# Julian-Wyatt/AnoDDPM

Hardware: AMD Instinct MI355X
Metric: reverse-diffusion images/sec @256x256 T=1000 simplex (higher is better)
Workload: dtype f32; 1 GPU; 256x256 simplex(8 oct) T=1000 base128 attn16,8 batch4/GPU (BASELINE config 2); per_gpu_batch=4, global_batch=4, T=1000, parallelism=batch-sharded x1 (no data-path collective), output_finite=True

## Files before the change

### anoddpm_amd/csrc/executor.hip

```cpp
#include <stdarg.h>
#include <string.h>
#include <vector>
#include "common.h"

namespace anoddpm {

static thread_local char g_err[512] = "";
int g_debug[16] = {0};

void set_error(const char *fmt, ...)
{
    va_list ap;
    va_start(ap, fmt);
    vsnprintf(g_err, sizeof(g_err), fmt, ap);
    va_end(ap);
}

struct ProfState {
    bool on = false;
    std::vector<hipEvent_t> pool;
    std::vector<int> codes;
    std::vector<float> last_ms;
    std::vector<int> last_codes;
    size_t used = 0;
// ... 7 lines not shown
    X(GN_STATS,         anoddpm_gn_args,               anoddpm_gn_stats) \
    X(SOFTMAX,          anoddpm_softmax_args,          anoddpm_softmax_rows) \
    X(RESAMPLE,         anoddpm_resample_args,         anoddpm_resample2x) \
    X(LINEAR,           anoddpm_linear_args,           anoddpm_linear_small) \
    X(POSEMB,           anoddpm_posemb_args,           anoddpm_posemb) \
    X(STEM,             anoddpm_stem_args,             anoddpm_conv_stem) \
    X(LAYOUT,           anoddpm_layout_args,           anoddpm_nhwc_to_nchw) \
    X(CHAN_STATS,       anoddpm_chan_stats_args,       anoddpm_chan_stats) \
    X(HEAD,             anoddpm_head_args,             anoddpm_conv_head) \
    X(GN_FINALIZE,      anoddpm_gn_finalize_args,      anoddpm_gn_finalize) \
    X(WGRAD3,           anoddpm_wgrad_args,            anoddpm_conv3x3_wgrad) \
    X(WGRAD1,           anoddpm_wgrad1_args,           anoddpm_wgrad_pointwise) \
    X(GN_BWD,           anoddpm_gn_bwd_args,           anoddpm_gn_silu_backward) \
    X(PACK,             anoddpm_pack_args,             anoddpm_pack_weights) \
    X(SOFTMAX_BWD,      anoddpm_softmax_bwd_args,      anoddpm_softmax_rows_backward) \
    X(TRANSPOSE,        anoddpm_transpose_args,        anoddpm_transpose_square) \
    X(LINEAR_BWD,       anoddpm_linear_bwd_args,       anoddpm_linear_small_backward) \
    X(STEM_BWD,         anoddpm_stem_bwd_args,         anoddpm_conv_stem_backward) \
    X(HEAD_BWD,         anoddpm_head_bwd_args,         anoddpm_conv_head_backward) \
    X(COLSUM_FOLD,      anoddpm_colsum_fold_args,      anoddpm_colsum_fold) \
    X(ATTENTION,        anoddpm_attention_args,        anoddpm_attention) \
    X(PACK_BATCH,       anoddpm_pack_batch_args,       anoddpm_pack_batch) \
    X(DROPOUT,          anoddpm_dropout_args,          anoddpm_dropout) \
    X(LINEAR_BWD_BATCH, anoddpm_linear_bwd_batch_args, anoddpm_linear_small_backward_batch)

static int dispatch(const anoddpm_op &op, void *stream)
{
    switch (op.code) {
#define X(code, args_t, fn) case ANODDPM_OP_##code: return fn(static_cast<const args_t *>(op.args), stream);
        ANODDPM_OPS(X)
#undef X
        default: set_error("run_ops: unknown op code %d", op.code); return ANODDPM_EINVAL;
    }
}

}

using namespace anoddpm;

extern "C" int anoddpm_internal_variant(int32_t key, int32_t value)
{
    if (key < 0 || key >= 16) return ANODDPM_EINVAL;
#ifndef ANODDPM_ABLATE
    if (!(key == 0 || key == 4 || key == 5 || key == 8 || key == 9)) {
        set_error("internal_variant: key %d selects a timing ablation; this library was built without ANODDPM_ABLATE", key);
        return ANODDPM_EINVAL;
    }
// ... 98 lines not shown
extern "C" int anoddpm_prof_list(int32_t *codes, float *ms, int32_t cap)
{
    const int n = (int)g_prof.last_ms.size();
    for (int i = 0; i < n && i < cap; ++i) {
        if (codes) codes[i] = g_prof.last_codes[i];
        if (ms) ms[i] = g_prof.last_ms[i];
    }
    return n;
}

#define ANODDPM_STRUCTS(X) \
    X(anoddpm_simplex_args) X(anoddpm_p_update_args) X(anoddpm_igemm_args) X(anoddpm_gn_args) X(anoddpm_softmax_args) \
    X(anoddpm_resample_args) X(anoddpm_linear_args) X(anoddpm_posemb_args) X(anoddpm_stem_args) X(anoddpm_layout_args) \
    X(anoddpm_op) X(anoddpm_adamw_args) X(anoddpm_chan_stats_args) X(anoddpm_gn_finalize_args) X(anoddpm_head_args) \
    X(anoddpm_anomaly_args) X(anoddpm_vlb_args) X(anoddpm_wgrad_args) X(anoddpm_gn_bwd_args) X(anoddpm_wgrad1_args) \
    X(anoddpm_pack_args) X(anoddpm_softmax_bwd_args) X(anoddpm_transpose_args) X(anoddpm_linear_bwd_args) \
    X(anoddpm_stem_bwd_args) X(anoddpm_head_bwd_args) X(anoddpm_colsum_fold_args) X(anoddpm_mri_slice_args) \
    X(anoddpm_resize_args) X(anoddpm_attention_args) X(anoddpm_pack_batch_args) X(anoddpm_linear_bwd_batch_args) \
    X(anoddpm_loss_args) X(anoddpm_dropout_args) X(anoddpm_roc_args) X(anoddpm_ssim_args) X(anoddpm_component_areas_args) \
    X(anoddpm_pro_args) X(anoddpm_distance_args) X(anoddpm_surface_args) X(anoddpm_median_args) X(anoddpm_erode_args) \
    X(anoddpm_components_args) X(anoddpm_gauss_args) X(anoddpm_map_scores_args) \
    X(anoddpm_ano_slices_args) X(anoddpm_select_args) X(anoddpm_threshold_counts_args) X(anoddpm_known_args) \
    X(anoddpm_resampling_args) X(anoddpm_keep_mask_args) X(anoddpm_median3d_args) X(anoddpm_erode3d_args) \
    X(anoddpm_components3d_args) X(anoddpm_component_areas3d_args) X(anoddpm_distance3d_args) X(anoddpm_surface3d_args)

extern "C" int anoddpm_struct_size(const char *name)
{
    if (reinterpret_cast<uintptr_t>(name) < 4096) return -1;
#define X(s) if (strcmp(name, #s) == 0) return (int)sizeof(s);
    ANODDPM_STRUCTS(X)
#undef X
    return -1;
}
```

### anoddpm_amd/csrc/simplex.hip

```cpp
#include "common.h"
#include "simplex_tables.h"

namespace {

constexpr double STRETCH3 = -1.0 / 6;
constexpr double SQUISH3 = 1.0 / 3;
constexpr double NORM3 = 103.0;


constexpr unsigned H_ENTRY0 = 2048, G_DELTA = 6144;
struct Tables {
    double grad[24][6];
    unsigned char pad0[H_ENTRY0 - 8 - 24 * 48];
    uint2 H[516];
    unsigned lut[REGION_LUT_SIZE];
    unsigned char pad1[G_DELTA - 516 * 8 - REGION_LUT_SIZE * 4];
    uint2 G[516];
    alignas(16) double vtx[128][10];
};
static_assert(offsetof(Tables, vtx) % 16 == 0, "vertex rows 16-byte aligned");
static_assert(offsetof(Tables, vtx) == VTX_LDS_BASE, "kRegionLutAddr holds addresses relative to this base");
static_assert(offsetof(Tables, lut) % 8 == 0 && REGION_LUT_SIZE % 2 == 0, "lut copied as 8-byte words");
static_assert(offsetof(Tables, H) == H_ENTRY0 - 8, "H entry 0 at byte 2048");
static_assert(offsetof(Tables, G) == H_ENTRY0 - 8 + G_DELTA, "G entry 0 at byte 2048 + 6144");
// ... 164 lines not shown
    if (pow2) {
        double rf = 1.0 / f0;
        for (int o = 0; o < octaves; ++o) {
            const double n = noise3<ABL, SAFE>(T, xd * rf, yd * rf, zd * rf);
            acc = acc + amp * n;
            rf = rf * 2.0;
            amp = amp * persistence;
        }
    } else {
        double f = f0;
        for (int o = 0; o < octaves; ++o) {
            const double n = noise3<ABL, SAFE>(T, xd / f, yd / f, zd / f);
            acc = acc + amp * n;
            f = f / 2;
            amp = amp * persistence;
        }
    }
    return acc;
}

#ifndef SIMPLEX_WAVES
#define SIMPLEX_WAVES 6
#endif
template <typename OutT, int ABL = 0>
__global__ __launch_bounds__(256) __attribute__((amdgpu_waves_per_eu(SIMPLEX_WAVES))) void simplex3_octaves_kernel(anoddpm_simplex_args a, int rows_per_block)
{
    __shared__ Tables T;
    const int s = blockIdx.z;
    long long tab = (a.table_sel ? (long long)(*a.table_sel) * a.table_sel_scale : 0) +
                    (long long)s * a.table_slice_stride;
    load_tables(T, a.tables + tab * 512);

    const int x = blockIdx.x * 64 + (threadIdx.x & 63);
    if (x >= a.W) return;
    const long long zi = a.zvals ? a.zvals[s] : a.z0 + s;

    const double f0 = a.frequency;
    int fe;
    const bool pow2 = (frexp(f0, &fe) == 0.5) && fe > -900 && fe - a.octaves > -900 && fe < 900;
    const double xd = (double)x, zd = (double)zi;
    const double fmin = ldexp(f0, -(a.octaves > 0 ? a.octaves - 1 : 0));
    for (int ty = 0; ty < rows_per_block; ++ty) {
        const int y = (blockIdx.y * rows_per_block + ty) * 4 + (threadIdx.x >> 6);
        if (y >= a.H) break;
        const double yd = (double)y;
        const bool safe = fmin > 0.0 && fmax(fmax(fabs(xd), fabs(yd)), fabs(zd)) * 2.0 < 2147483000.0 * fmin;
        double acc = 0.0;
        if (safe) acc = octave_sum<ABL, true>(T, xd, yd, zd, f0, pow2, a.octaves, a.persistence);
        else      acc = octave_sum<ABL, false>(T, xd, yd, zd, f0, pow2, a.octaves, a.persistence);
        OutT *out = reinterpret_cast<OutT *>(a.out) + (long long)s * a.out_slice_stride + (long long)y * a.W + x;
        *out = (OutT)acc;
    }
}

__global__ __launch_bounds__(256) void simplex3_grid_kernel(double *out, const double *X, int nx, const double *Y, int ny,
                                                            const double *Z, int nz, const int16_t *tables)
{
    __shared__ Tables T;
    load_tables(T, tables);
    const long long total = (long long)nx * ny * nz;
    for (long long i = (long long)blockIdx.x * 256 + threadIdx.x; i < total; i += (long long)gridDim.x * 256) {
        const int ix = (int)(i % nx);
        const int iy = (int)((i / nx) % ny);
        const int iz = (int)(i / ((long long)nx * ny));
        out[i] = noise3<0>(T, X[ix], Y[iy], Z[iz]);
    }
}

constexpr double STRETCH2 = -0.211324865405187;
constexpr double SQUISH2 = 0.366025403784439;
constexpr double NORM2 = 47.0;
__constant__ signed char kGrad2[16] = {5, 2, 2, 5, -5, 2, -2, 5, 5, -2, 2, -5, -5, -2, -2, -5};

struct Tables2 {
// ... 102 lines not shown
    const uint64_t MUL = 6364136223846793005ULL, INC = 1442695040888963407ULL;
    for (int w = 0; w < 3; ++w) s = s * MUL + INC;
    for (int i = 255; i >= 0; --i) {
        s = s * MUL + INC;
        __int128 wide = (__int128)(int64_t)s + 31;
        __int128 m = wide % (i + 1);
        if (m < 0) m += i + 1;
        const int r = (int)m;
        perm[i] = source[r];
        pgi3[i] = (int16_t)((perm[i] % 24) * 3);
        source[r] = source[i];
    }
    return ANODDPM_OK;
}

template <typename OutT>
static int launch_simplex(const anoddpm_simplex_args *a, void *stream)
{
    ANODDPM_REQUIRE(a && a->out && a->tables, "simplex3_octaves: null pointer");
    ANODDPM_REQUIRE(a->nslices >= 0 && a->H >= 0 && a->W >= 0 && a->octaves >= 0, "simplex3_octaves: negative size");
    ANODDPM_REQUIRE(a->nslices <= 65535, "simplex3_octaves: nslices > 65535 (split the launch)");
    ANODDPM_REQUIRE(a->out_slice_stride >= (int64_t)a->H * a->W, "simplex3_octaves: slice stride < H*W");
    if (a->nslices == 0 || a->H == 0 || a->W == 0) return ANODDPM_OK;
    const long long tiles = (long long)((a->W + 63) / 64) * ((a->H + 3) / 4) * a->nslices;
    const int rpb = tiles >= 4ll * 8 * 1536 ? 4 : (tiles >= 2ll * 8 * 1536 ? 2 : 1);
    dim3 grid((a->W + 63) / 64, ((a->H + 3) / 4 + rpb - 1) / rpb, a->nslices);
    ANODDPM_REQUIRE(grid.y <= 65535, "simplex3_octaves: H too large");
#ifdef ANODDPM_ABLATE
    const int abl = anoddpm::g_debug[7];
    if (abl == 1) hipLaunchKernelGGL((simplex3_octaves_kernel<OutT, 1>), grid, dim3(256), 0, anoddpm::as_stream(stream), *a, rpb);
    else if (abl == 2) hipLaunchKernelGGL((simplex3_octaves_kernel<OutT, 2>), grid, dim3(256), 0, anoddpm::as_stream(stream), *a, rpb);
    else if (abl == 3) hipLaunchKernelGGL((simplex3_octaves_kernel<OutT, 3>), grid, dim3(256), 0, anoddpm::as_stream(stream), *a, rpb);
    else
#endif
    hipLaunchKernelGGL((simplex3_octaves_kernel<OutT, 0>), grid, dim3(256), 0, anoddpm::as_stream(stream), *a, rpb);
    return anoddpm::check_launch("simplex3_octaves");
}

extern "C" int anoddpm_simplex3_octaves_f64(const anoddpm_simplex_args *a, void *stream)
{
    return launch_simplex<double>(a, stream);
}

extern "C" int anoddpm_simplex3_octaves_f32(const anoddpm_simplex_args *a, void *stream)
{
    return launch_simplex<float>(a, stream);
// ... 27 lines not shown
```

### anoddpm_amd/csrc/unet_kernels.hip

```cpp
#include "common.h"
#include "gn_stats.h"

using anoddpm::gn_affine;
using anoddpm::gn_moments;
using anoddpm::gf_f32x4;
using anoddpm::silu_f;
using anoddpm::slab_column_sums;

namespace {

__global__ __launch_bounds__(256) void gn_partial_kernel(anoddpm_gn_args a)
{
    __shared__ double lds_s[256 * 4];
    __shared__ double lds_q[256 * 4];
    const int C = a.c0 + a.c1;
    const int C4 = C >> 2;
    const int TQ = C4 < 256 ? C4 : 256;
    const int R = 256 / TQ;
    const int npass = (C4 + TQ - 1) / TQ;
    const int cpg = C / a.groups;
    const int tid = threadIdx.x;
    const int tq = tid % TQ, tr = tid / TQ;
    const int b = blockIdx.y, slab = blockIdx.x;
    const int sp = (a.P + a.nslab - 1) / a.nslab;
// ... 292 lines not shown
                float v = acc[b] + bias;
                if (a.act_out) v = silu_f(v);
                a.out[(int64_t)b * a.N + n] = v;
            }
        }
    }
}

__global__ void posemb_kernel(anoddpm_posemb_args a)
{
    const int half = a.dim >> 1;
    const int i = blockIdx.x * blockDim.x + threadIdx.x;
    for (int64_t z = (int64_t)i * 2; z < a.zero_doubles; z += (int64_t)gridDim.x * blockDim.x * 2) {
        a.zero[z] = 0.0;
        if (z + 1 < a.zero_doubles) a.zero[z + 1] = 0.0;
    }
    if (i >= a.B * half) return;
    const int b = i / half, j = i % half;
    const float arg = ((float)a.t[b] * a.scale) * a.freqs[j];
    a.out[(int64_t)b * a.dim + j] = sinf(arg);
    a.out[(int64_t)b * a.dim + half + j] = cosf(arg);
}

constexpr int STEM_STRIP = 8;

template <int CIN>
__global__ __launch_bounds__(256) void conv_stem_strip2_kernel(anoddpm_stem_args a)
{
    __shared__ float lds_s[256 * 4];
    __shared__ float lds_q[256 * 4];
    const int QP = a.Cout >> 2;
    const int spb = 256 / QP;
    const int q = threadIdx.x % QP;
    const int sl = threadIdx.x / QP;
    const bool lane_on = sl < spb;
    const int strips_x = a.W / STEM_STRIP;
    const int64_t nstrips = (int64_t)a.B * a.H * strips_x;
    const int64_t strip0 = (int64_t)blockIdx.x * spb * 2;
    const float4 *w = reinterpret_cast<const float4 *>(a.w);
    float4 wr[9 * CIN];
#pragma unroll
    for (int t = 0; t < 9; ++t)
#pragma unroll
        for (int ci = 0; ci < CIN; ++ci) wr[t * CIN + ci] = w[(t * CIN + ci) * QP + (lane_on ? q : 0)];
    const float4 bias = a.bias ? reinterpret_cast<const float4 *>(a.bias)[lane_on ? q : 0] : make_float4(0.f, 0.f, 0.f, 0.f);
    float4 ssum = make_float4(0.f, 0.f, 0.f, 0.f), ssq = make_float4(0.f, 0.f, 0.f, 0.f);
// ... 613 lines not shown
        anoddpm_linear_args c = *a;
        c.in = a->in + (int64_t)b0 * a->K;
        c.out = a->out + (int64_t)b0 * a->N;
        c.B = a->B - b0 < 16 ? a->B - b0 : 16;
        if (c.B <= 4) hipLaunchKernelGGL(linear_small_kernel<4>, grid, dim3(256), 0, s, c);
        else if (c.B <= 8) hipLaunchKernelGGL(linear_small_kernel<8>, grid, dim3(256), 0, s, c);
        else hipLaunchKernelGGL(linear_small_kernel<16>, grid, dim3(256), 0, s, c);
    }
    return anoddpm::check_launch("linear_small");
}

extern "C" int anoddpm_posemb(const anoddpm_posemb_args *a, void *stream)
{
    ANODDPM_REQUIRE(a && a->t && a->freqs && a->out && a->B >= 1 && a->dim >= 2 && a->dim % 2 == 0, "posemb: bad arguments");
    const int n = a->B * (a->dim / 2);
    ANODDPM_REQUIRE(a->zero_doubles >= 0 && (a->zero_doubles == 0 || (a->zero && (uintptr_t)a->zero % 8 == 0)), "posemb: bad zero range");
    int64_t blocks = (n + 255) / 256;
    const int64_t zblocks = (a->zero_doubles / 2 + 255) / 256;
    if (zblocks > blocks) blocks = zblocks < 512 ? zblocks : 512;
    hipLaunchKernelGGL(posemb_kernel, dim3((unsigned)blocks), dim3(256), 0, anoddpm::as_stream(stream), *a);
    return anoddpm::check_launch("posemb");
}

extern "C" int anoddpm_stem_stats_rows(int H, int W, int Cin, int Cout)
{
    if (Cin < 1 || Cin > 2 || W <= 0 || H <= 0 || W % STEM_STRIP || Cout <= 0 || Cout % 4 || Cout / 4 > 256) return 0;
    const int ppb = 256 / (Cout / 4);
    const int64_t per_image = (int64_t)H * W / STEM_STRIP;
    if (per_image % ppb) return 0;
    const int64_t trips = per_image / ppb;
    int64_t iters = 1;
    if (anoddpm::g_debug[9] != 1 && Cin == 1 && trips % 2 == 0 && trips / 2 >= 256) iters = 2;
    while (trips / iters > 1024) iters *= 2;
    while (iters > 1 && trips % iters) iters /= 2;
    return (int)(trips / iters);
}

extern "C" int anoddpm_conv_stem(const anoddpm_stem_args *a, void *stream)
{
    ANODDPM_REQUIRE(a && a->x && a->w && a->out, "conv_stem: null pointer");
    ANODDPM_REQUIRE(a->Cin >= 1 && a->Cin <= 16 && a->Cout % 4 == 0 && a->Cout / 4 <= 256, "conv_stem: need Cin<=16, Cout%%4==0, Cout<=1024");
    const int ppb = 256 / (a->Cout / 4);
    const int64_t npix = (int64_t)a->B * a->H * a->W;
    if (npix == 0) return ANODDPM_OK;
    if (a->Cin <= 2 && a->W % STEM_STRIP == 0 && (uintptr_t)a->x % 16 == 0) {
        const int64_t nstrips = npix / STEM_STRIP;
// ... 75 lines not shown
```

### anoddpm_amd/diffusion.py

```python
import ctypes
import random

import numpy as np
import torch

from . import _lib, philox
from ._lib import KnownArgs, LossArgs, PUpdateArgs, ResamplingArgs, VlbArgs, check, current_stream, lib, ptr
from .simplex import Simplex_CLASS, perm_tables

__all__ = ["SimplexNoiseFn", "GaussNoiseFn", "ReverseChain", "StridedSampler", "KnownRegion", "Resampling", "get_beta_schedule", "extract", "mean_flat", "normal_kl", "approx_standard_normal_cdf",
           "discretised_gaussian_log_likelihood", "generate_simplex_noise", "random_noise",
           "GaussianDiffusionModel"]

_RANDOM_PARAMS = [(2, 0.6, 16), (6, 0.6, 32), (7, 0.7, 32), (10, 0.8, 64), (5, 0.8, 16), (4, 0.6, 16),
                  (1, 0.6, 64), (7, 0.8, 128), (6, 0.9, 64), (2, 0.85, 128), (2, 0.85, 64), (2, 0.85, 32),
                  (2, 0.85, 16), (2, 0.85, 8), (2, 0.85, 4), (2, 0.85, 2), (1, 0.85, 128), (1, 0.85, 64),
                  (1, 0.85, 32), (1, 0.85, 16), (1, 0.85, 8), (1, 0.85, 4), (1, 0.85, 2)]


def get_beta_schedule(num_diffusion_steps, name="cosine"):
    if name == "cosine":
        def abar(u):
            return np.cos((u + 0.008) / 1.008 * np.pi / 2) ** 2
        n = num_diffusion_steps
# ... 281 lines not shown
    for i, (slot, start) in enumerate(place):
        refill.setdefault(start, []).append((slot, i))
        harvest.setdefault(start + steps[i] - 1, []).append((slot, i))
        last_busy[slot] = max(last_busy[slot], start + steps[i])
    return refill, harvest, last_busy


class ReverseChain:

    def __init__(self, owner, model, x, t_distance, denoise_fn, use_graph=None, stream_base=None, sampler=None, known=None,
                 resampling=None, shared_planes=False):
        _lib.require_cuda(x, "ReverseChain")
        self.owner, self.model, self.denoise_fn = owner, model, denoise_fn
        import os
        self.graph = None
        self._graph_state = 0
        self.B = x.shape[0]
        self.x = torch.empty(x.shape, device=x.device, dtype=torch.float32)
        self.t = torch.empty((self.B,), device=x.device, dtype=torch.int64)
        self.step_idx = torch.empty(1, device=x.device, dtype=torch.int32)
        self.sampler = _check_sampler(sampler)
        self.hip_model = hasattr(model, "forward_hip") and not self._draws_dropout(model)
        self._plan = None
        self.noise = None
        self.tables = None
        fn, capture_safe = self._resolve_noise(owner, denoise_fn)
        if isinstance(fn, SimplexNoiseFn):
            self.simplex_fn = fn
            self.noise = torch.empty_like(self.x)
            self.tables = torch.empty((owner.num_timesteps * fn.in_channels, 512), dtype=torch.int16, device=x.device)
        self.resampling = self._check_resample_request(owner, denoise_fn, sampler, known, resampling)
        self.reuse_key = self._reuse_key_of(owner, denoise_fn, sampler, known, resampling, shared_planes)
        self.capture_safe = capture_safe
        self.known_mode = self._known_mode_of(owner, denoise_fn, known)
        self.k_x0 = self.k_keep = self.k_noise = None
        self.shared_planes = bool(shared_planes) and self.known_mode is not None
        if self.known_mode is not None:
            plane = (1,) + tuple(x.shape[1:]) if self.shared_planes else tuple(x.shape)
            self.k_x0 = torch.empty(plane, device=x.device, dtype=torch.float32)
            self.k_keep = torch.empty(plane, device=x.device, dtype=torch.uint8)
            if self.known_mode == "fixed":
                self.k_noise = torch.empty_like(self.x)
        self.rs_top = self.rs_rep = self.rs_visit = self.rs_jump = self.rs_reps = None
        if self.resampling is not None:
            self.rs_top, self.rs_rep, self.rs_visit = (torch.empty((self.B,), dtype=torch.int32, device=x.device) for _ in range(3))
            self.rs_jump, self.rs_reps = (torch.empty(1, dtype=torch.int32, device=x.device) for _ in range(2))
# ... 150 lines not shown
            self.rs_jump.fill_(self.resampling.jump)
            self.rs_reps.fill_(self.resampling.reps)
        if self.sampler is not None:
            self.owner._sampler_words(self.x.device, self.sampler)
        if self.tables is not None:
            self._draw_tables(self.remaining)
        if self.streams is not None:
            self._set_streams(stream_base)
        if known is not None:
            self.k_x0.copy_(known.x_0)
            self.k_keep.copy_(known.keep)
            if self.k_noise is not None:
                if torch.is_tensor(known.noise):
                    self.k_noise.copy_(known.noise)
                elif int(t_distance) > 0 and not self.shared_planes:
                    t_top = torch.full((self.B,), int(t_distance) - 1, device=self.x.device, dtype=torch.int64)
                    self.k_noise.copy_(self.owner.noise_fn(self.k_x0, t_top).float())

    def step(self):
        if self.sampler is not None:
            self.owner._sampler_words(self.x.device, self.sampler)
        if self.use_graph and lib().anoddpm_prof_active() == 0:
            if self._graph_state == 2:
                self.graph.replay()
                self.remaining -= 1
                return self.x
            if self._graph_state == 1:
                torch.cuda.synchronize()
                if self.hip_model:
                    self._plan = self.model._plan_for(self.B, self.x.shape[2], self.x.device)
                g = torch.cuda.CUDAGraph()
                import gc
                gc.collect()
                gc.collect()
                gc_was_enabled = gc.isenabled()
                gc.disable()
                try:
                    with torch.cuda.graph(g):
                        self._step_body()
                finally:
                    if gc_was_enabled:
                        gc.enable()
                self.graph = g
                self._graph_state = 2
                g.replay()
                self.remaining -= 1
                return self.x
            self._graph_state = 1
        self._step_body()
        self.remaining -= 1
        return self.x

    def _step_body(self):
        o = self.owner

        with torch.no_grad():
            eps = self.model.forward_hip(self.x, self.t, borrow=True) if self.hip_model else self.model(self.x, self.t)
            if self.tables is not None:
                fn = self.simplex_fn
                for c in range(fn.in_channels):
                    fn.simplex.fill_fixed_T_octaves_(self.noise, self.t, fn.octave, fn.persistence, fn.frequency,
                                                     channel=c, tables=self.tables[c:], table_sel=self.step_idx,
                                                     table_sel_scale=fn.in_channels)
                noise = self.noise
            elif self.streams is not None:
                noise = None
            else:
                noise = o._denoise_noise(self.x, self.t, self.denoise_fn)
            words = o._sampler_words(self.x.device, None) if self.sampler is not None else None
            if self.resampling is not None:
                renoise = torch.randn_like(self.x) if self.streams is None else None
                state = (self.rs_jump, self.rs_reps, self.rs_top, self.rs_rep, self.rs_visit)
                o._known_update(self.x, self.t, eps, noise, (self.k_x0, self.k_keep, self.k_noise), None, want_pred=False,
                                out=self.x, gauss_streams=self.streams, resample=state + (renoise,))
                check(lib().anoddpm_chain_advance_resample(ptr(self.t), self.B, ptr(self.step_idx), *(ptr(w) for w in state),
                                                           current_stream()), "chain_advance_resample")
                return
            if self.known_mode is not None:
                o._known_update(self.x, self.t, eps, noise, (self.k_x0, self.k_keep, self.k_noise), words, want_pred=False,
                                out=self.x, gauss_streams=self.streams)
            elif self.sampler is not None:
                o._strided_update(self.x, self.t, eps, noise, None, want_pred=False, out=self.x, gauss_streams=self.streams)
            else:
                o._reverse_update(self.x, self.t, eps, noise, want_pred=False, out=self.x, gauss_streams=self.streams)
            if self.sampler is not None:
                check(lib().anoddpm_chain_advance_strided(ptr(self.t), self.B, ptr(self.step_idx), ptr(words.stride),
# ... 888 lines not shown
```

### anoddpm_amd/simplex.py

```python
import ctypes

import numpy as np
import torch

from . import _lib
from ._lib import SimplexArgs, check, current_stream, lib, ptr

__all__ = ["Simplex_CLASS", "perm_tables"]


def _wrap64(seed):
    return ((int(seed) + (1 << 63)) % (1 << 64)) - (1 << 63)


def perm_tables(seed):
    tab = np.zeros(512, dtype=np.int16)
    p = tab.ctypes.data_as(ctypes.POINTER(ctypes.c_int16))
    check(lib().anoddpm_simplex_perm_init(_wrap64(seed), p, ctypes.cast(ctypes.addressof(p.contents) + 512, ctypes.POINTER(ctypes.c_int16))),
          "simplex_perm_init")
    return tab


def _device():
    if not torch.cuda.is_available():
# ... 2 lines not shown


class Simplex_CLASS:

    def __init__(self):
        self._dev_tables = None
        self.newSeed()

    def newSeed(self, seed=None):
        if not seed:
            seed = np.random.randint(-10000000000, 10000000000)
        self._tables = perm_tables(seed)
        self._perm = self._tables[:256].astype(np.int64)
        self._perm_grad_index3 = self._tables[256:].astype(np.int64)
        self._dev_tables = None

    def device_tables(self, device=None):
        device = device or _device()
        if self._dev_tables is None or self._dev_tables.device != device:
            self._dev_tables = torch.from_numpy(self._tables).to(device)
        return self._dev_tables

    def fill_fixed_T_octaves_(self, out, t, octaves=1, persistence=0.5, frequency=32, channel=0,
                              tables=None, table_sel=None, table_sel_scale=1):
        _lib.require_cuda(out, "Simplex_CLASS.fill_fixed_T_octaves_")
        assert out.dtype == torch.float32 and out.is_contiguous() and out.dim() == 4
        B, C, H, W = out.shape
        if t.dtype != torch.int64 or t.device != out.device:
            t = t.to(device=out.device, dtype=torch.int64)
        t = t.contiguous()
        assert t.numel() == B
        tab = tables if tables is not None else self.device_tables(out.device)
        a = SimplexArgs()
        a.out = out.data_ptr() + 4 * channel * H * W
        a.zvals = t.data_ptr()
        a.tables = tab.data_ptr()
        a.table_sel = table_sel.data_ptr() if table_sel is not None else None
        a.z0 = 0
        a.out_slice_stride = C * H * W
        a.nslices, a.H, a.W = B, H, W
        a.table_slice_stride = 0
        a.table_sel_scale = table_sel_scale
        a.octaves = int(octaves)
        a.persistence = float(persistence)
        a.frequency = float(frequency)
        check(lib().anoddpm_simplex3_octaves_f32(ctypes.byref(a), current_stream()), "simplex3_octaves_f32")
        return out

    def _octaves_f64(self, zvals, z0, nslices, H, W, octaves, persistence, frequency):
        dev = _device()
        out = torch.empty((nslices, H, W), dtype=torch.float64, device=dev)
        if out.numel() == 0 or octaves <= 0:
            return out.zero_().cpu().numpy()
        a = SimplexArgs()
        a.out = out.data_ptr()
        zt = None
        if zvals is not None:
            zt = torch.from_numpy(np.ascontiguousarray(zvals, dtype=np.int64)).to(dev)
            a.zvals = zt.data_ptr()
        a.tables = self.device_tables(dev).data_ptr()
        a.table_sel = None
        a.z0 = int(z0)
        a.out_slice_stride = H * W
        a.H, a.W = H, W
        a.table_slice_stride = 0
        a.table_sel_scale = 1
        a.octaves = int(octaves)
        a.persistence = float(persistence)
# ... 62 lines not shown
```

### anoddpm_amd/unet.py

```python
import ctypes
import math
import os
from types import SimpleNamespace

import numpy as np
import torch
from torch import nn

from . import _lib
from ._lib import (AttentionArgs, ChanStatsArgs, GnFinalizeArgs, HeadArgs, IgemmArgs, LayoutArgs, LinearArgs, Op, PackArgs, PackBatchArgs,
                   PosembArgs, ResampleArgs, SoftmaxArgs, StemArgs, check, lib)

__all__ = ["UNetModel", "update_ema_params", "zero_module", "GroupNorm32"]

_DEFAULT_MULTS = {512: (0.5, 1, 1, 2, 2, 4, 4), 256: (1, 1, 2, 2, 4, 4), 128: (1, 1, 2, 3, 4),
                  64: (1, 2, 3, 4), 32: (1, 2, 3, 4)}


class _Affine(nn.Module):

    def __init__(self, c):
        super().__init__()
        self.weight = nn.Parameter(torch.ones(c))
        self.bias = nn.Parameter(torch.zeros(c))


class _Weights(nn.Module):

    def __init__(self, shape, zero=False):
        super().__init__()
        self.weight = nn.Parameter(torch.empty(*shape))
        self.bias = nn.Parameter(torch.empty(shape[0]))
        nn.init.kaiming_uniform_(self.weight, a=math.sqrt(5))
# ... 199 lines not shown

    def _forward_train_mode_no_grad(self, x, time):
        _lib.require_cuda(x, "UNetModel.forward (train mode)")
        if not (x.dim() == 4 and x.shape[2] == x.shape[3] and x.shape[1] == self.in_channels):
            raise ValueError(f"expected [B,{self.in_channels},S,S] input, got {tuple(x.shape)}")
        from . import train_plan
        B, S = x.shape[0], x.shape[2]
        if not train_plan.eligible(self, B, S):
            raise NotImplementedError(f"UNetModel in train() mode with dropout at batch {B}, size {S}: outside the native training plan; "
                                      "call .eval() for sampling")
        plan = self._train_plan_for(B, S, x.device, False, float(self.dropout))
        xin = x.detach()
        if xin.dtype != torch.float32 or not xin.is_contiguous():
            xin = xin.float().contiguous()
        if xin.data_ptr() % 16:
            xin = xin.clone()
        t = time.detach()
        if t.dtype != torch.int64 or t.device != x.device or not t.is_contiguous():
            t = t.to(device=x.device, dtype=torch.int64).contiguous()
        y = plan.run_forward(xin, t)
        plan.fwd_epoch = getattr(plan, "fwd_epoch", 0) + 1
        return y.clone().to(x.dtype)

    def forward_hip(self, x, time, out=None, borrow=False):
        _lib.require_cuda(x, "UNetModel.forward")
        B, C, H, W = x.shape
        if C != self.in_channels or H != W:
            raise ValueError(f"expected [B,{self.in_channels},S,S] input, got {tuple(x.shape)}")
        plan = self._plan_for(B, H, x.device)
        xin = x.detach()
        if xin.dtype != torch.float32 or not xin.is_contiguous():
            xin = xin.float().contiguous()
        if xin.data_ptr() % 16:
            xin = xin.clone()
        t = time.detach()
        if t.dtype != torch.int64 or t.device != x.device or not t.is_contiguous():
            t = t.to(device=x.device, dtype=torch.int64).contiguous()
        y = plan.run(xin, t)
        if out is not None:
            out.copy_(y.view_as(out))
            return out
        if borrow and x.dtype == torch.float32:
            return y.view_as(x)
        return y.clone().to(x.dtype)

    def _plan_for(self, B, S, device):
        key = (B, S, device, os.environ.get("ANODDPM_ARITH", "fp32"))
        plan = self._plans.get(key)
        if plan is None:
            plan = _Plan(self, B, S, device)
            self._plans[key] = plan
        plan.refresh_weights()
        return plan

    def _train_plan_for(self, B, S, device, want_dx, p_drop=0.0):
        from .train_plan import TrainPlan
        key = (B, S, device, bool(want_dx), float(p_drop))
        plan = self._tplans.get(key)
        if plan is None or not plan.params_match():
            plan = self._tplans[key] = TrainPlan(self, B, S, device, want_dx=want_dx, p_drop=p_drop)
        return plan
# ... 209 lines not shown
        self._bf16_jobs = []
        self._packed = {}
        self.arith = os.environ.get("ANODDPM_ARITH", "fp32") if self.honours_arith else "fp32"
        if self.arith not in ("fp32", "bf16split3"):
            raise ValueError(f"ANODDPM_ARITH={self.arith}: expected fp32 or bf16split3")
        self.token = None
        self.igemm_flops = 0.0
        self._ws_need = 0
        self.stats_of = {}
        self.igemm_log = []
        self.block_out = {}
        self.csum_mode = self.honours_csum and os.environ.get("ANODDPM_CSUM", "0") == "1"
        self._csum_arena, self._csum_used = None, 0
        if self.csum_mode:
            cap = 2 * B * sum(p.shape[0] for p in model.parameters() if p.dim() == 4 and p.shape[-1] == 3)
            self._csum_arena = torch.zeros(max(cap, 2), dtype=torch.float64, device=device)
            self.keep.append(self._csum_arena)
        with torch.no_grad():
            self._build()
        if self.csum_mode and getattr(self, "posemb", None) is not None:
            self.posemb.zero = self._csum_arena.data_ptr() if self._csum_used else None
            self.posemb.zero_doubles = self._csum_used
        self.op_array = _op_array(self.ops)

    def buf(self, *shape, dtype=torch.float32):
        t = torch.empty(*shape, dtype=dtype, device=self.device)
        self.keep.append(t)
        return t

    def packed(self, key, kind, out=None):
        ck = (key, kind, None if out is None else out.data_ptr())
        hit = self._packed.get(ck)
        if hit is not None:
            return hit
        p = dict(self.model.named_parameters())[key]
        shape = tuple(p.shape)
        if kind == "wino43b":
            N, K = shape[0], shape[1]
            dst = torch.empty(54 * N * K, dtype=torch.float32, device=self.device)
            self.keep.append(dst)
            self._bf16_jobs.append((key, dst, N, K))
            self._packed[ck] = dst
            return dst
        k = pack_kind(kind, shape)
        N, K = (p.numel(), 1) if k == PACK_KINDS["copy"] else (shape[0], shape[1])
        n_out = pack_floats(k, N, K)
# ... 12 lines not shown
        self.ops.append((code, st))
        return st

    def refresh_weights(self):
        params = list(self.model.parameters())
        token = (self.model._weights_epoch,) + tuple((p.data_ptr(), p._version) for p in params)
        if token == self.token:
            return
        named = dict(self.model.named_parameters())
        for key, st in self._pack_jobs:
            src = named[key]
            if src.device != self.device:
                raise _lib.AnoddpmError(f"parameter {key} is on {src.device}, plan is on {self.device}")
            if src.dtype != torch.float32 or not src.is_contiguous():
                raise _lib.AnoddpmError(f"parameter {key} must be contiguous fp32")
            st.w = src.data_ptr()
        pb, raw, b0 = _pack_table([st for _, st in self._pack_jobs], self.device)
        check(lib().anoddpm_pack_batch(ctypes.byref(pb), _lib.current_stream()), "weight packing")
        for key, dst, N, K in self._bf16_jobs:
            check(lib().anoddpm_pack_wino43_bf16x3(named[key].data_ptr(), dst.data_ptr(), N, K, _lib.current_stream()), "bf16 weight planes")
        self._pack_table = (raw, b0, pb)
        self.token = token
        self.pack_count = getattr(self, "pack_count", 0) + 1

    def chan_stats(self, buf, C, P):
        B = self.B
        nslab = max(1, min(128, (P * (C // 4)) // 4096))
        stats = self.buf(B, nslab, C, 2)
        st = ChanStatsArgs()
        st.a, st.stats, st.a_bs = buf.data_ptr(), stats.data_ptr(), P * C
        st.C, st.a_ld, st.P, st.B, st.nslab = C, C, P, B, nslab
        self.add(_lib.OP_CHAN_STATS, st)
        self.stats_of[buf.data_ptr()] = _Stats("rows", stats, nslab)

    fuse_gn_tail = True

    def stats_source(self, st, which, src, c):
        ptr, rows, fmt = self.stats_of[src.data_ptr()].triple()
        setattr(st, f"stats{which}", ptr)
        setattr(st, f"rows{which}", rows)
        setattr(st, f"fmt{which}", fmt)

    def gn_tail_job(self, srcs, gamma, beta, want_mean=False):
        B = self.B
        c0 = srcs[0][1]
        c1 = srcs[1][1] if len(srcs) > 1 else 0
# ... 414 lines not shown
            else:
                self.y = self.buf(B, nout, S, S)
                st = LayoutArgs()
                st.inp, st.out, st.B, st.P, st.C, st.in_ld = y_nhwc.data_ptr(), self.y.data_ptr(), B, S * S, nout, nout
                self.add(_lib.OP_LAYOUT, st)
        return SimpleNamespace(x=hfin, C=cfin, g=g, nout=nout)

    def run_blocks(self, blks, srcs, Hc):
        for (prefix, kind, cin, cout, resample) in blks:
            if kind == "stem":
                r = self.stem_block(prefix, cin, cout)
            elif kind == "res":
                r = self.res_block(prefix, srcs, Hc, cout, resample)
            elif kind in ("downsample", "upsample"):
                r = self.resample_layer(prefix, kind, srcs[0][0], Hc, cin, resample == "conv")
            else:
                r = self.attn_block(prefix, srcs[0][0], Hc, cin)
            srcs, Hc = [(r.out, r.C)], r.H
            self.block_out[prefix] = (r.out, r.C, Hc)
        return srcs, Hc

    def walk(self):
        self.time_path()
        down, middle, up = self.model._blocks
        Hc, srcs, skips = self.S, None, []
        for blk in down:
            srcs, Hc = self.run_blocks(blk, srcs, Hc)
            skips.append(srcs[0])
        srcs, Hc = self.run_blocks(middle, srcs, Hc)
        for blk in up:
            srcs, Hc = self.run_blocks(blk, [srcs[0], skips.pop()], Hc)
        return self.head_block(*srcs[0])

    def share_workspace(self, ops):
        if self._ws_need:
            ws = self.buf(self._ws_need)
            for code, st in ops:
                if code == _lib.OP_IGEMM and st.ksplit > 1:
                    st.ws = ws.data_ptr()

    def _build(self):
        self.walk()
        self.share_workspace(self.ops)

    def run(self, x, t):
        self.stem.x = x.data_ptr()
        self.posemb.t = t.data_ptr()
        check(lib().anoddpm_run_ops(self.op_array, len(self.ops), _lib.current_stream()), "UNet forward")
        return self.y
```

### include/anoddpm_hip.h

```cpp
#ifndef ANODDPM_HIP_H
#define ANODDPM_HIP_H

#include <stdint.h>

#ifdef __cplusplus
extern "C" {
#endif

#define ANODDPM_OK 0
#define ANODDPM_EINVAL (-1)
#define ANODDPM_ELAUNCH (-2)
#define ANODDPM_ENODEV (-3)

#define ANODDPM_ABI_VERSION 42

int anoddpm_abi_version(void);
const char *anoddpm_last_error(void);
int anoddpm_device_count(void);
int anoddpm_struct_size(const char *name);


int anoddpm_simplex_perm_init(int64_t seed, int16_t *perm, int16_t *pgi3);

typedef struct {
    void *out;
    const int64_t *zvals;
    const int16_t *tables;
    const int32_t *table_sel;
    int64_t z0;
    int64_t out_slice_stride;
    int32_t nslices, H, W;
    int32_t table_slice_stride;
    int32_t table_sel_scale;
    int32_t octaves;
    double persistence;
    double frequency;
} anoddpm_simplex_args;

int anoddpm_simplex3_octaves_f64(const anoddpm_simplex_args *a, void *stream);
int anoddpm_simplex3_octaves_f32(const anoddpm_simplex_args *a, void *stream);

int anoddpm_simplex3_grid_f64(double *out, const double *X, int32_t nx, const double *Y, int32_t ny,
                              const double *Z, int32_t nz, const int16_t *tables, void *stream);

int anoddpm_simplex2_octaves_f64(double *out, int32_t n, const int16_t *tables, int32_t octaves,
                                 double persistence, double frequency, void *stream);
int anoddpm_simplex2_grid_f64(double *out, const double *X, const double *Y, int32_t n, const int16_t *tables,
                              void *stream);


int anoddpm_q_sample(float *out, const float *x, const float *noise, const int64_t *t,
                     const float *ca, const float *cb, int32_t B, int64_t n, int32_t T,
                     void *stream);

typedef struct {
    float *x_prev;
    float *pred_x0;
    float *mean_out;
    const float *x_t;
// ... 41 lines not shown
    ANODDPM_OP_SOFTMAX = 3,
    ANODDPM_OP_RESAMPLE = 4,
    ANODDPM_OP_LINEAR = 5,
    ANODDPM_OP_POSEMB = 6,
    ANODDPM_OP_STEM = 7,
    ANODDPM_OP_LAYOUT = 8,
    ANODDPM_OP_CHAN_STATS = 9,
    ANODDPM_OP_GN_FINALIZE = 10,
    ANODDPM_OP_HEAD = 11,
    ANODDPM_OP_WGRAD3 = 16,
    ANODDPM_OP_WGRAD1 = 17,
    ANODDPM_OP_GN_BWD = 18,
    ANODDPM_OP_PACK = 19,
    ANODDPM_OP_SOFTMAX_BWD = 20,
    ANODDPM_OP_TRANSPOSE = 21,
    ANODDPM_OP_LINEAR_BWD = 22,
    ANODDPM_OP_STEM_BWD = 23,
    ANODDPM_OP_HEAD_BWD = 24,
    ANODDPM_OP_COLSUM_FOLD = 25,
    ANODDPM_OP_ATTENTION = 26,
    ANODDPM_OP_PACK_BATCH = 27,
    ANODDPM_OP_LINEAR_BWD_BATCH = 28,
    ANODDPM_OP_DROPOUT = 29,
    ANODDPM_OP_MAX = 32
};

typedef struct {
    const float *a0, *a1;
    const float *gn_scale, *gn_shift;
    const float *bmat;
    const float *bias;
    const float *temb;
    const float *res;
    float *out;
    float *ws;
    int64_t a0_bs, a0_hs, a1_bs, a1_hs;
    int64_t b_bs, b_hs;
    int64_t o_bs, o_hs, r_bs, r_hs;
    int32_t c0, c1;
    int32_t a0_ld, a1_ld;
    int32_t H, W;
    int32_t ks;
    int32_t a_mode;
    int32_t act;
    int32_t b_mode;
    int32_t ldb;
// ... 110 lines not shown
    const float *in;
    const float *w;
    const float *bias;
    float *out;
    int32_t B, K, N;
    int32_t act_in, act_out;
} anoddpm_linear_args;

int anoddpm_linear_small(const anoddpm_linear_args *a, void *stream);

typedef struct {
    const int64_t *t;
    const float *freqs;
    float *out;
    int32_t B, dim;
    float scale;
    double *zero;
    int64_t zero_doubles;
} anoddpm_posemb_args;

int anoddpm_posemb(const anoddpm_posemb_args *a, void *stream);

typedef struct {
    const float *x;
    const float *w;
    const float *bias;
    float *out;
    int32_t B, H, W, Cin, Cout;
    float *stats;
    int32_t stats_rows;
} anoddpm_stem_args;

int anoddpm_stem_stats_rows(int H, int W, int Cin, int Cout);

int anoddpm_conv_stem(const anoddpm_stem_args *a, void *stream);

typedef struct {
    const float *x;
    const float *w;
    const float *bias;
    const float *gn_scale, *gn_shift;
    float *out;
    int32_t B, H, W, C, Cout;
} anoddpm_head_args;

int anoddpm_conv_head(const anoddpm_head_args *a, void *stream);
// ... 648 lines not shown
```

Baseline: 0.4560 images/s.

## Precompute timestep embedding table and broadcast one simplex noise field across batch

Adds a per-T table of the full time-embedding path outputs (posemb plus MLPs), built eagerly for all timesteps and gathered per step by a new EMB_GATHER op that replaces the time-path ops in the UNet op list. Simplex noise generation gains a broadcast mode that computes one field and writes it to every batch slice when the batch shares a timestep, cutting the simplex work by the batch size. The table costs memory and a rebuild whenever weights are repacked. Broadcast mode relies on all slots sharing the same noise tables, and graphs captured in that mode cannot be replayed as slot chains.

```diff
diff --git a/anoddpm_amd/csrc/executor.hip b/anoddpm_amd/csrc/executor.hip
--- a/anoddpm_amd/csrc/executor.hip
+++ b/anoddpm_amd/csrc/executor.hip
@@ -53,7 +53,8 @@
     X(ATTENTION,        anoddpm_attention_args,        anoddpm_attention) \
     X(PACK_BATCH,       anoddpm_pack_batch_args,       anoddpm_pack_batch) \
     X(DROPOUT,          anoddpm_dropout_args,          anoddpm_dropout) \
-    X(LINEAR_BWD_BATCH, anoddpm_linear_bwd_batch_args, anoddpm_linear_small_backward_batch)
+    X(LINEAR_BWD_BATCH, anoddpm_linear_bwd_batch_args, anoddpm_linear_small_backward_batch) \
+    X(EMB_GATHER,       anoddpm_emb_gather_args,       anoddpm_emb_gather)
 
 static int dispatch(const anoddpm_op &op, void *stream)
 {
@@ -198,7 +199,8 @@
     X(anoddpm_components_args) X(anoddpm_gauss_args) X(anoddpm_map_scores_args) \
     X(anoddpm_ano_slices_args) X(anoddpm_select_args) X(anoddpm_threshold_counts_args) X(anoddpm_known_args) \
     X(anoddpm_resampling_args) X(anoddpm_keep_mask_args) X(anoddpm_median3d_args) X(anoddpm_erode3d_args) \
-    X(anoddpm_components3d_args) X(anoddpm_component_areas3d_args) X(anoddpm_distance3d_args) X(anoddpm_surface3d_args)
+    X(anoddpm_components3d_args) X(anoddpm_component_areas3d_args) X(anoddpm_distance3d_args) X(anoddpm_surface3d_args) \
+    X(anoddpm_emb_gather_args)
 
 extern "C" int anoddpm_struct_size(const char *name)
 {
diff --git a/anoddpm_amd/csrc/simplex.hip b/anoddpm_amd/csrc/simplex.hip
--- a/anoddpm_amd/csrc/simplex.hip
+++ b/anoddpm_amd/csrc/simplex.hip
@@ -210,11 +210,11 @@
 #ifndef SIMPLEX_WAVES
 #define SIMPLEX_WAVES 6
 #endif
-template <typename OutT, int ABL = 0>
+template <typename OutT, int ABL = 0, bool BCAST = false>
 __global__ __launch_bounds__(256) __attribute__((amdgpu_waves_per_eu(SIMPLEX_WAVES))) void simplex3_octaves_kernel(anoddpm_simplex_args a, int rows_per_block)
 {
     __shared__ Tables T;
-    const int s = blockIdx.z;
+    const int s = BCAST ? 0 : blockIdx.z;
     long long tab = (a.table_sel ? (long long)(*a.table_sel) * a.table_sel_scale : 0) +
                     (long long)s * a.table_slice_stride;
     load_tables(T, a.tables + tab * 512);
@@ -238,6 +238,8 @@
         else      acc = octave_sum<ABL, false>(T, xd, yd, zd, f0, pow2, a.octaves, a.persistence);
         OutT *out = reinterpret_cast<OutT *>(a.out) + (long long)s * a.out_slice_stride + (long long)y * a.W + x;
         *out = (OutT)acc;
+        if (BCAST)
+            for (int p = 1; p < a.nslices; ++p) out[(long long)p * a.out_slice_stride] = (OutT)acc;
     }
 }
 
@@ -386,6 +388,13 @@
     ANODDPM_REQUIRE(a->nslices <= 65535, "simplex3_octaves: nslices > 65535 (split the launch)");
     ANODDPM_REQUIRE(a->out_slice_stride >= (int64_t)a->H * a->W, "simplex3_octaves: slice stride < H*W");
     if (a->nslices == 0 || a->H == 0 || a->W == 0) return ANODDPM_OK;
+    ANODDPM_REQUIRE(a->broadcast == 0 || a->broadcast == 1, "simplex3_octaves: broadcast must be 0 or 1");
+    if (a->broadcast) {
+        dim3 bgrid((a->W + 63) / 64, (a->H + 3) / 4, 1);
+        ANODDPM_REQUIRE(bgrid.y <= 65535, "simplex3_octaves: H too large");
+        hipLaunchKernelGGL((simplex3_octaves_kernel<OutT, 0, true>), bgrid, dim3(256), 0, anoddpm::as_stream(stream), *a, 1);
+        return anoddpm::check_launch("simplex3_octaves");
+    }
     const long long tiles = (long long)((a->W + 63) / 64) * ((a->H + 3) / 4) * a->nslices;
     const int rpb = tiles >= 4ll * 8 * 1536 ? 4 : (tiles >= 2ll * 8 * 1536 ? 2 : 1);
     dim3 grid((a->W + 63) / 64, ((a->H + 3) / 4 + rpb - 1) / rpb, a->nslices);
diff --git a/anoddpm_amd/csrc/unet_kernels.hip b/anoddpm_amd/csrc/unet_kernels.hip
--- a/anoddpm_amd/csrc/unet_kernels.hip
+++ b/anoddpm_amd/csrc/unet_kernels.hip
@@ -338,6 +338,23 @@
     a.out[(int64_t)b * a.dim + half + j] = cosf(arg);
 }
 
+__global__ __launch_bounds__(256) void emb_gather_kernel(anoddpm_emb_gather_args a)
+{
+    const int i = blockIdx.x * blockDim.x + threadIdx.x;
+    for (int64_t z = (int64_t)i * 2; z < a.zero_doubles; z += (int64_t)gridDim.x * blockDim.x * 2) {
+        a.zero[z] = 0.0;
+        if (z + 1 < a.zero_doubles) a.zero[z + 1] = 0.0;
+    }
+    const int n4 = a.n >> 2;
+    if (i >= a.B * n4) return;
+    const int b = i / n4, j = i % n4;
+    const int64_t t = a.t[b];
+    const float qnan = __int_as_float(0x7fc00000);
+    float4 v = make_float4(qnan, qnan, qnan, qnan);
+    if (t >= 0 && t < a.T) v = reinterpret_cast<const float4 *>(a.table + t * a.n)[j];
+    reinterpret_cast<float4 *>(a.out + (int64_t)b * a.n)[j] = v;
+}
+
 constexpr int STEM_STRIP = 8;
 
 template <int CIN>
@@ -997,6 +1014,21 @@
     return anoddpm::check_launch("posemb");
 }
 
+extern "C" int anoddpm_emb_gather(const anoddpm_emb_gather_args *a, void *stream)
+{
+    ANODDPM_REQUIRE(a && a->t && a->table && a->out, "emb_gather: null pointer");
+    ANODDPM_REQUIRE(a->B >= 1 && a->T >= 1 && a->n >= 4 && a->n % 4 == 0, "emb_gather: need B >= 1, T >= 1, n %% 4 == 0");
+    ANODDPM_REQUIRE((int64_t)a->B * (a->n / 4) <= 0x7fffffff, "emb_gather: B * n too large");
+    ANODDPM_REQUIRE((uintptr_t)a->table % 16 == 0 && (uintptr_t)a->out % 16 == 0, "emb_gather: table and out must be 16-byte aligned");
+    ANODDPM_REQUIRE(a->zero_doubles >= 0 && (a->zero_doubles == 0 || (a->zero && (uintptr_t)a->zero % 8 == 0)), "emb_gather: bad zero range");
+    int64_t blocks = ((int64_t)a->B * (a->n / 4) + 255) / 256;
+    int64_t zblocks = (a->zero_doubles / 2 + 255) / 256;
+    if (zblocks > 512) zblocks = 512;
+    if (zblocks > blocks) blocks = zblocks;
+    hipLaunchKernelGGL(emb_gather_kernel, dim3((unsigned)blocks), dim3(256), 0, anoddpm::as_stream(stream), *a);
+    return anoddpm::check_launch("emb_gather");
+}
+
 extern "C" int anoddpm_stem_stats_rows(int H, int W, int Cin, int Cout)
 {
     if (Cin < 1 || Cin > 2 || W <= 0 || H <= 0 || W % STEM_STRIP || Cout <= 0 || Cout % 4 || Cout / 4 > 256) return 0;
diff --git a/anoddpm_amd/diffusion.py b/anoddpm_amd/diffusion.py
--- a/anoddpm_amd/diffusion.py
+++ b/anoddpm_amd/diffusion.py
@@ -327,6 +327,8 @@
         self.sampler = _check_sampler(sampler)
         self.hip_model = hasattr(model, "forward_hip") and not self._draws_dropout(model)
         self._plan = None
+        self.slot_chain = False
+        self._captured_broadcast = False
         self.noise = None
         self.tables = None
         fn, capture_safe = self._resolve_noise(owner, denoise_fn)
@@ -523,6 +525,9 @@
             self.owner._sampler_words(self.x.device, self.sampler)
         if self.use_graph and lib().anoddpm_prof_active() == 0:
             if self._graph_state == 2:
+                if self.slot_chain and self._captured_broadcast:
+                    raise ValueError("ReverseChain: this chain's graph was captured with one noise field for the whole batch; "
+                                     "it cannot be replayed as a slot chain with per-slot timesteps")
                 self.graph.replay()
                 self.remaining -= 1
                 return self.x
@@ -556,13 +561,18 @@
         o = self.owner
 
         with torch.no_grad():
-            eps = self.model.forward_hip(self.x, self.t, borrow=True) if self.hip_model else self.model(self.x, self.t)
+            eps = (self.model.forward_hip(self.x, self.t, borrow=True, timesteps=o.num_timesteps, t_in_range=True)
+                   if self.hip_model else self.model(self.x, self.t))
             if self.tables is not None:
                 fn = self.simplex_fn
+                import os
+                broadcast = self.B > 1 and not self.slot_chain and os.environ.get("ANODDPM_NO_NOISE_BCAST", "0") != "1"
+                if torch.cuda.is_current_stream_capturing():
+                    self._captured_broadcast = broadcast
                 for c in range(fn.in_channels):
                     fn.simplex.fill_fixed_T_octaves_(self.noise, self.t, fn.octave, fn.persistence, fn.frequency,
                                                      channel=c, tables=self.tables[c:], table_sel=self.step_idx,
-                                                     table_sel_scale=fn.in_channels)
+                                                     table_sel_scale=fn.in_channels, broadcast=broadcast)
                 noise = self.noise
             elif self.streams is not None:
                 noise = None
diff --git a/anoddpm_amd/simplex.py b/anoddpm_amd/simplex.py
--- a/anoddpm_amd/simplex.py
+++ b/anoddpm_amd/simplex.py
@@ -48,7 +48,7 @@
         return self._dev_tables
 
     def fill_fixed_T_octaves_(self, out, t, octaves=1, persistence=0.5, frequency=32, channel=0,
-                              tables=None, table_sel=None, table_sel_scale=1):
+                              tables=None, table_sel=None, table_sel_scale=1, broadcast=False):
         _lib.require_cuda(out, "Simplex_CLASS.fill_fixed_T_octaves_")
         assert out.dtype == torch.float32 and out.is_contiguous() and out.dim() == 4
         B, C, H, W = out.shape
@@ -70,6 +70,7 @@
         a.octaves = int(octaves)
         a.persistence = float(persistence)
         a.frequency = float(frequency)
+        a.broadcast = 1 if broadcast else 0
         check(lib().anoddpm_simplex3_octaves_f32(ctypes.byref(a), current_stream()), "simplex3_octaves_f32")
         return out
 
diff --git a/anoddpm_amd/unet.py b/anoddpm_amd/unet.py
--- a/anoddpm_amd/unet.py
+++ b/anoddpm_amd/unet.py
@@ -8,7 +8,7 @@
 from torch import nn
 
 from . import _lib
-from ._lib import (AttentionArgs, ChanStatsArgs, GnFinalizeArgs, HeadArgs, IgemmArgs, LayoutArgs, LinearArgs, Op, PackArgs, PackBatchArgs,
+from ._lib import (AttentionArgs, ChanStatsArgs, EmbGatherArgs, GnFinalizeArgs, HeadArgs, IgemmArgs, LayoutArgs, LinearArgs, Op, PackArgs, PackBatchArgs,
                    PosembArgs, ResampleArgs, SoftmaxArgs, StemArgs, check, lib)
 
 __all__ = ["UNetModel", "update_ema_params", "zero_module", "GroupNorm32"]
@@ -254,7 +254,7 @@
         plan.fwd_epoch = getattr(plan, "fwd_epoch", 0) + 1
         return y.clone().to(x.dtype)
 
-    def forward_hip(self, x, time, out=None, borrow=False):
+    def forward_hip(self, x, time, out=None, borrow=False, timesteps=None, t_in_range=False):
         _lib.require_cuda(x, "UNetModel.forward")
         B, C, H, W = x.shape
         if C != self.in_channels or H != W:
@@ -268,7 +268,10 @@
         t = time.detach()
         if t.dtype != torch.int64 or t.device != x.device or not t.is_contiguous():
             t = t.to(device=x.device, dtype=torch.int64).contiguous()
-        y = plan.run(xin, t)
+        if timesteps is not None and not t_in_range:
+            if torch.cuda.is_current_stream_capturing() or not bool(((t >= 0) & (t < int(timesteps))).all()):
+                timesteps = None
+        y = plan.run(xin, t, timesteps)
         if out is not None:
             out.copy_(y.view_as(out))
             return out
@@ -524,6 +527,9 @@
             self.posemb.zero = self._csum_arena.data_ptr() if self._csum_used else None
             self.posemb.zero_doubles = self._csum_used
         self.op_array = _op_array(self.ops)
+        self.computed = (self.ops, self.op_array)
+        self._emb_tables = {}
+        self.emb_gathers = self.emb_computed = 0
 
     def buf(self, *shape, dtype=torch.float32):
         t = torch.empty(*shape, dtype=dtype, device=self.device)
@@ -582,6 +588,8 @@
         self._pack_table = (raw, b0, pb)
         self.token = token
         self.pack_count = getattr(self, "pack_count", 0) + 1
+        for ent in getattr(self, "_emb_tables", {}).values():
+            self._fill_emb_table(ent)
 
     def chan_stats(self, buf, C, P):
         B = self.B
@@ -1042,6 +1050,7 @@
 
     def walk(self):
         self.time_path()
+        self._n_time_ops = len(self.ops)
         down, middle, up = self.model._blocks
         Hc, srcs, skips = self.S, None, []
         for blk in down:
@@ -1063,8 +1072,53 @@
         self.walk()
         self.share_workspace(self.ops)
 
-    def run(self, x, t):
+    def emb_table(self, T):
+        ent = self._emb_tables.get(T)
+        if ent is None:
+            ent = SimpleNamespace(T=T, table=self.buf(T, self._emb_tot), pack_count=None, builds=0)
+            ent.t_all = torch.arange(-(-T // self.B) * self.B, device=self.device, dtype=torch.int64).clamp_(max=T - 1).view(-1, self.B)
+            self.keep.append(ent.t_all)
+            st = EmbGatherArgs()
+            st.t, st.table, st.out = None, ent.table.data_ptr(), self._emb_all.data_ptr()
+            st.B, st.T, st.n = self.B, T, self._emb_tot
+            st.zero, st.zero_doubles = self.posemb.zero, self.posemb.zero_doubles
+            self.keep.append(st)
+            ent.gather = st
+            ent.ops = [(_lib.OP_EMB_GATHER, st)] + self.computed[0][self._n_time_ops:]
+            ent.op_array = _op_array(ent.ops)
+            self._emb_tables[T] = ent
+        if ent.pack_count != getattr(self, "pack_count", 0):
+            self._fill_emb_table(ent)
+        return ent
+
+    def _fill_emb_table(self, ent):
+        if torch.cuda.is_current_stream_capturing():
+            raise _lib.AnoddpmError("the embedding table must be built outside a stream capture (run one eager step first)")
+        ops, arr = self.computed
+        held = self.posemb.t
+        for i in range(ent.t_all.shape[0]):
+            self.posemb.t = ent.t_all[i].data_ptr()
+            check(lib().anoddpm_run_ops(arr, self._n_time_ops, _lib.current_stream()), "embedding table")
+            rows = min(self.B, ent.T - i * self.B)
+            ent.table[i * self.B:i * self.B + rows].copy_(self._emb_all[:rows])
+        self.posemb.t = held
+        ent.pack_count = getattr(self, "pack_count", 0)
+        ent.builds += 1
+
+    def emb_table_usable(self):
+        return (os.environ.get("ANODDPM_NO_EMB_TABLE", "0") != "1" and self._emb_tot % 4 == 0
+                and self._emb_all.data_ptr() % 16 == 0)
+
+    def run(self, x, t, timesteps=None):
         self.stem.x = x.data_ptr()
-        self.posemb.t = t.data_ptr()
+        if timesteps is not None and self.emb_table_usable():
+            ent = self.emb_table(int(timesteps))
+            ent.gather.t = t.data_ptr()
+            self.ops, self.op_array = ent.ops, ent.op_array
+            self.emb_gathers += 1
+        else:
+            self.posemb.t = t.data_ptr()
+            self.ops, self.op_array = self.computed
+            self.emb_computed += 1
         check(lib().anoddpm_run_ops(self.op_array, len(self.ops), _lib.current_stream()), "UNet forward")
         return self.y
diff --git a/include/anoddpm_hip.h b/include/anoddpm_hip.h
--- a/include/anoddpm_hip.h
+++ b/include/anoddpm_hip.h
@@ -12,7 +12,7 @@
 #define ANODDPM_ELAUNCH (-2)
 #define ANODDPM_ENODEV (-3)
 
-#define ANODDPM_ABI_VERSION 42
+#define ANODDPM_ABI_VERSION 43
 
 int anoddpm_abi_version(void);
 const char *anoddpm_last_error(void);
@@ -35,6 +35,7 @@
     int32_t octaves;
     double persistence;
     double frequency;
+    int32_t broadcast;
 } anoddpm_simplex_args;
 
 int anoddpm_simplex3_octaves_f64(const anoddpm_simplex_args *a, void *stream);
@@ -122,6 +123,7 @@
     ANODDPM_OP_PACK_BATCH = 27,
     ANODDPM_OP_LINEAR_BWD_BATCH = 28,
     ANODDPM_OP_DROPOUT = 29,
+    ANODDPM_OP_EMB_GATHER = 30,
     ANODDPM_OP_MAX = 32
 };
 
@@ -278,6 +280,17 @@
 int anoddpm_posemb(const anoddpm_posemb_args *a, void *stream);
 
 typedef struct {
+    const int64_t *t;
+    const float *table;
+    float *out;
+    int32_t B, T, n;
+    double *zero;
+    int64_t zero_doubles;
+} anoddpm_emb_gather_args;
+
+int anoddpm_emb_gather(const anoddpm_emb_gather_args *a, void *stream);
+
+typedef struct {
     const float *x;
     const float *w;
     const float *bias;
```

Result: no change. 0.4575 images/s (median of 6 runs) (+0.3%).
